# al-mcintyre/mCaller

Measured on NVIDIA B200. Metric: per-read site calls/sec, higher is better.
Workload: dtype f64

## Files before the change

### include/mcaller_b200.h

```cpp
#ifndef MCALLER_B200_H
#define MCALLER_B200_H

#include <stdint.h>

#ifdef __cplusplus
extern "C" {
#endif

#define MC_ABI_VERSION 3

#define MC_TILE_BYTES 3840
#define MC_TEXT_PAD 4096
#define MC_MAXK 8

enum {
    MC_OK = 0,
    MC_EINVAL = -1,
    MC_ECUDA = -2,
    MC_ECAPACITY = -3
};

typedef struct mc_refindex {
    int32_t n_contigs;
    int32_t k;
    const uint8_t *d_names;
    const int32_t *d_name_off;
    const int64_t *d_base;
    const int32_t *d_len;
    const uint32_t *d_site_fwd;
    const uint32_t *d_site_rev;
    const uint32_t *d_cand;
    const uint32_t *d_rank_fwd;
    const uint32_t *d_rank_rev;
    const uint8_t *d_bases;
    int64_t total_bits;
} mc_refindex;

typedef struct mc_record {
    uint32_t line_lo;
    uint16_t line_hi;
    uint16_t name_off;
    int32_t pos;
    int32_t event_idx;
    double diff;
    uint16_t name_len;
    uint16_t contig;
    uint8_t flags;
    uint8_t kbits_fwd;
    uint8_t kbits_rev;
    uint8_t pad;
} mc_record;

#define MC_RF_EQ 1u
#define MC_RF_CAND 2u
#define MC_RF_BADNUM 4u
#define MC_RF_BADIDX 8u
#define MC_RF_RAW 16u
#define MC_RF_NEWREAD 32u
#define MC_RF_SEGKNOWN 64u

enum {
    MC_C_LINES = 0,
    MC_C_KEPT,
    MC_C_RECORDS,
    MC_C_SHORT,
    MC_C_UNKNOWN_CONTIG,
    MC_C_NNN,
    MC_C_BADPOS,
    MC_C_LONGLINE,
    MC_C_OVERFLOW,
    MC_C_RUN_CURSOR,
    MC_C_QUIET,
    MC_C_COUNT = 16
};

typedef struct mc_call {
    int64_t read_off;
    double prob;
    double feat[MC_MAXK + 1];
    int32_t read_len;
    int32_t mpos;
    int32_t site;
    uint32_t close_rec;
    uint16_t win_contig;
    uint16_t chrom_contig;
    uint8_t kind;
    uint8_t rev;
    uint8_t n_empty;
    uint8_t empty_mask;
    uint8_t model_sel;
    uint8_t label;
    uint8_t err;
    uint8_t pad0;
    uint32_t seg;
    uint32_t pad1;
    uint32_t pad2;
} mc_call;

enum { MC_CALL = 0, MC_TOO_MANY_SKIPS = 1, MC_MULTI_M = 2, MC_NONE = 3  };
#define MC_CE_CONTEXT 1u
#define MC_CE_MODELKEY 2u
#define MC_CE_BADNUM 4u
#define MC_CE_COLUMN 8u
#define MC_CE_SPACING 16u

enum { MC_MLP = 0, MC_LR = 1, MC_GNB = 2, MC_RF = 3 };
enum { MC_ACT_IDENTITY = 0, MC_ACT_LOGISTIC = 1, MC_ACT_TANH = 2, MC_ACT_RELU = 3 };
typedef struct mc_model {
    int32_t kind;
    int32_t n_in;
    int32_t n_layers;
    int32_t hidden_act;
    int32_t sizes[8];
    const double *d_weights;
    const double *d_biases;
    int32_t n_trees;
    int32_t max_nodes;
    const int32_t *d_tree_off;
    const int32_t *d_left;
    const int32_t *d_right;
    const int32_t *d_feature;
    const double *d_threshold;
    const double *d_leaf_p1;
} mc_model;

typedef struct mc_qual_entry {
    uint64_t hash;
    uint32_t check;
    uint32_t len;
    double qual;
} mc_qual_entry;


int mc_version(void);
int mc_sizeof(int what);
const char *mc_last_error(void);

int mc_read_u64(const uint64_t *d_src, int64_t n, uint64_t *h_dst, void *stream);

int mc_scan(const uint8_t *d_text, int64_t nbytes, const mc_refindex *ref, int dense,
            mc_record *d_rec, int64_t rec_cap, uint32_t *d_tile_tab , uint32_t *d_run_tab ,
            uint64_t *d_counters, void *stream);

int mc_scan_run_len(int64_t nbytes);

int mc_scan_set_run_len(int run_len);

int64_t mc_num_tiles(int64_t nbytes);

int64_t mc_workspace_bytes(int64_t n);

int mc_order_records(const uint8_t *d_text, int64_t nbytes, const mc_refindex *ref, const uint32_t *d_tile_tab, int64_t n_tiles,
                     uint32_t *d_run_tab, int run_len, const mc_record *d_rec_in, int64_t rec_in_cap, const uint64_t *d_scan_counters,
                     mc_record *d_rec_out, int64_t rec_out_cap, uint64_t *d_n_out, uint32_t *d_seg_flags ,
                     uint32_t *d_run_first , void *d_ws, void *stream);

int mc_segment_reads(const uint8_t *d_text, mc_record *d_rec, const uint64_t *d_n_records, int64_t rec_cap,
                     uint32_t *d_seg_flags , const uint32_t *d_run_first, int64_t n_runs,
                     uint32_t *d_seg_start, uint64_t *d_nseg, void *d_ws, void *stream);

int mc_segment_quality(const uint8_t *d_text, const mc_record *d_rec, const uint32_t *d_seg_start, const uint64_t *d_nseg,
                       int64_t seg_cap, const mc_qual_entry *d_table, int64_t table_size, double *d_seg_qual, uint64_t *d_err,
                       void *stream);

int mc_build_windows(const mc_record *d_rec, const uint64_t *d_n_records, int64_t rec_cap, const uint32_t *d_seg_start,
                     const uint64_t *d_nseg, int64_t seg_cap, const double *d_seg_qual, const mc_refindex *ref, int skip_thresh,
                     double qual_thresh, int two_models, mc_call *d_calls, int64_t call_cap, uint32_t *d_seg_count,
                     uint64_t *d_ncalls, void *d_ws, double *d_spill, int64_t spill_cap, void *stream);

typedef struct mc_carry {
    mc_call row;
    uint32_t valid;
    int32_t first_kept_contig;
    uint64_t chunks;
    uint64_t pad[6];
} mc_carry;
int mc_carry_reset(mc_carry *d_carry, void *stream);
int mc_carry_rows(mc_call *d_rows, const uint64_t *d_ncalls, const mc_record *d_rec, const uint64_t *d_n_records,
                  const uint32_t *d_seg_start, const uint64_t *d_nseg, const double *d_seg_qual, double qual_thresh,
                  mc_carry *d_carry, uint64_t *d_nrows_out, const uint64_t *d_abort, void *stream);
int mc_chunk_guard(const uint64_t *d_counters, int64_t rec_cap, const uint64_t *d_n_records, int64_t rec_out_cap,
                   const uint64_t *d_nseg, int64_t seg_cap, const uint64_t *d_ncalls, int64_t call_cap, uint64_t *d_abort,
                   uint64_t *d_sticky , void *stream);
int mc_carry_close(mc_carry *d_carry, int closing_contig, const int64_t *d_next_contigs, int from, int count, mc_call *d_row_out,
                   uint32_t *d_depth, uint32_t *d_meth, uint64_t *d_first, int64_t n_sites, uint64_t *d_row_base, void *stream);

int64_t mc_classify_workspace_bytes(int64_t row_cap);
int mc_classify(mc_call *d_calls, const uint64_t *d_nrows, int64_t row_cap, const mc_model *models, void *d_ws, void *stream);

int mc_hist_accumulate(const mc_call *d_calls, const uint64_t *d_nrows, int64_t row_cap, uint32_t *d_depth, uint32_t *d_meth,
                       uint64_t *d_first, int64_t n_sites, uint64_t *d_row_base, mc_call *d_odd, int64_t odd_cap, uint64_t *d_n_odd,
                       const uint64_t *d_abort , void *stream);

int mc_bed_select(const uint32_t *d_depth, const uint32_t *d_meth, int64_t n_sites, int64_t depth_thresh, double mod_thresh,
                  int control, uint8_t *d_flags, uint64_t *d_count, void *stream);

int mc_count_calls(const mc_call *d_calls, const uint64_t *d_nrows, int64_t row_cap, uint64_t *d_out, void *stream);

typedef struct mc_locus_entry {
    unsigned long long hash;
// ... 83 lines not shown
```

### mcaller_b200/_lib.py

```python
import ctypes as C
import os

import numpy as np

HERE = os.path.dirname(os.path.abspath(__file__))
LIB_PATH = os.environ.get("MCALLER_B200_LIB") or os.path.join(HERE, "libmcaller_b200.so")

MC_TILE_BYTES = 3840
MC_TEXT_PAD = 4096
MC_MAXK = 8
MC_C_COUNT = 16
COUNTER_NAMES = ["lines", "kept", "records", "short", "unknown_contig", "nnn", "badpos", "longline", "overflow", "run_cursor", "quiet_chunks"]

MC_ABI_VERSION = 3
MC_CALL, MC_TOO_MANY_SKIPS, MC_MULTI_M, MC_NONE = 0, 1, 2, 3
MC_CE_CONTEXT, MC_CE_MODELKEY, MC_CE_BADNUM, MC_CE_COLUMN, MC_CE_SPACING = 1, 2, 4, 8, 16
MC_MLP, MC_LR, MC_GNB, MC_RF = 0, 1, 2, 3
PENDING = 0xFFFFFFFF


class RefIndex(C.Structure):
    _fields_ = [("n_contigs", C.c_int32), ("k", C.c_int32), ("d_names", C.c_void_p), ("d_name_off", C.c_void_p),
                ("d_base", C.c_void_p), ("d_len", C.c_void_p), ("d_site_fwd", C.c_void_p), ("d_site_rev", C.c_void_p),
                ("d_cand", C.c_void_p), ("d_rank_fwd", C.c_void_p), ("d_rank_rev", C.c_void_p), ("d_bases", C.c_void_p),
                ("total_bits", C.c_int64)]


class Model(C.Structure):
    _fields_ = [("kind", C.c_int32), ("n_in", C.c_int32), ("n_layers", C.c_int32), ("hidden_act", C.c_int32),
                ("sizes", C.c_int32 * 8), ("d_weights", C.c_void_p), ("d_biases", C.c_void_p), ("n_trees", C.c_int32),
                ("max_nodes", C.c_int32), ("d_tree_off", C.c_void_p), ("d_left", C.c_void_p), ("d_right", C.c_void_p),
                ("d_feature", C.c_void_p), ("d_threshold", C.c_void_p), ("d_leaf_p1", C.c_void_p)]


class SynthSpec(C.Structure):
    _fields_ = [("seed", C.c_uint64), ("n_contigs", C.c_int32), ("len_min", C.c_int32), ("len_max", C.c_int32),
                ("p_skip", C.c_int32), ("p_nnn", C.c_int32), ("margin", C.c_int32), ("meth", C.c_int32),
                ("d_names", C.c_void_p), ("d_name_off", C.c_void_p), ("d_contig_len", C.c_void_p),
                ("d_read_bounds", C.c_void_p), ("d_gbase", C.c_void_p), ("d_genome", C.c_void_p),
                ("d_meth_fwd", C.c_void_p), ("d_meth_rev", C.c_void_p), ("d_model_mean", C.c_void_p),
                ("d_model_sd", C.c_void_p)]


RECORD_DTYPE = np.dtype([("line_lo", "<u4"), ("line_hi", "<u2"), ("name_off", "<u2"), ("pos", "<i4"), ("event_idx", "<i4"),
                         ("diff", "<f8"), ("name_len", "<u2"), ("contig", "<u2"), ("flags", "u1"), ("kbits_fwd", "u1"), ("kbits_rev", "u1"), ("pad", "u1")])
assert RECORD_DTYPE.itemsize == 32

CALL_DTYPE = np.dtype([("read_off", "<i8"), ("prob", "<f8"), ("feat", "<f8", (MC_MAXK + 1,)), ("read_len", "<i4"),
                       ("mpos", "<i4"), ("site", "<i4"), ("close_rec", "<u4"), ("win_contig", "<u2"), ("chrom_contig", "<u2"),
                       ("kind", "u1"), ("rev", "u1"), ("n_empty", "u1"), ("empty_mask", "u1"), ("model_sel", "u1"),
                       ("label", "u1"), ("err", "u1"), ("pad0", "u1"), ("seg", "<u4"), ("pad1", "<u4"), ("pad2", "<u4")])
assert CALL_DTYPE.itemsize == 128

class LocusEntry(C.Structure):
    _fields_ = [("hash", C.c_uint64), ("first_off", C.c_uint64), ("check", C.c_uint64), ("depth", C.c_uint32), ("meth", C.c_uint32)]


class TrainJob(C.Structure):
    _fields_ = [("d_x", C.c_void_p), ("d_y", C.c_void_p), ("d_w", C.c_void_p), ("d_loss_curve", C.c_void_p), ("idx_off", C.c_int64),
                ("n", C.c_int32), ("d", C.c_int32), ("max_iter", C.c_int32), ("n_iter_no_change", C.c_int32), ("alpha", C.c_double),
                ("lr", C.c_double), ("tol", C.c_double), ("best_loss", C.c_double), ("n_iter", C.c_int32), ("no_improve", C.c_int32),
                ("stopped", C.c_int32), ("pad", C.c_int32)]


MC_TRAIN_HIDDEN, MC_TRAIN_BATCH = 100, 200

CARRY_BYTES = 192

QUAL_DTYPE = np.dtype([("hash", "<u8"), ("check", "<u4"), ("len", "<u4"), ("qual", "<f8")])
assert QUAL_DTYPE.itemsize == 24
DIFFS_ROW_DTYPE = np.dtype([("line_off", "<u8"), ("slot", "<u4"), ("values_off", "<u4"), ("values_len", "<u4"), ("prob_off", "<u4"),
                            ("prob_len", "<u4"), ("pad", "<u4")])
assert DIFFS_ROW_DTYPE.itemsize == 32


class McallerCudaError(RuntimeError):
    pass


_lib = None

_PROTOS = {
    "mc_version": (C.c_int, []),
    "mc_sizeof": (C.c_int, [C.c_int]),
    "mc_last_error": (C.c_char_p, []),
    "mc_read_u64": (C.c_int, [C.c_void_p, C.c_int64, C.c_void_p, C.c_void_p]),
    "mc_scan": (C.c_int, [C.c_void_p, C.c_int64, C.POINTER(RefIndex), C.c_int, C.c_void_p, C.c_int64, C.c_void_p, C.c_void_p, C.c_void_p,
                          C.c_void_p]),
    "mc_scan_run_len": (C.c_int, [C.c_int64]),
    "mc_scan_set_run_len": (C.c_int, [C.c_int]),
    "mc_num_tiles": (C.c_int64, [C.c_int64]),
    "mc_workspace_bytes": (C.c_int64, [C.c_int64]),
    "mc_order_records": (C.c_int, [C.c_void_p, C.c_int64, C.POINTER(RefIndex), C.c_void_p, C.c_int64, C.c_void_p, C.c_int, C.c_void_p,
                                   C.c_int64, C.c_void_p, C.c_void_p, C.c_int64, C.c_void_p, C.c_void_p, C.c_void_p, C.c_void_p, C.c_void_p]),
    "mc_segment_reads": (C.c_int, [C.c_void_p, C.c_void_p, C.c_void_p, C.c_int64, C.c_void_p, C.c_void_p, C.c_int64, C.c_void_p, C.c_void_p,
                                   C.c_void_p, C.c_void_p]),
    "mc_segment_quality": (C.c_int, [C.c_void_p, C.c_void_p, C.c_void_p, C.c_void_p, C.c_int64, C.c_void_p, C.c_int64, C.c_void_p,
                                     C.c_void_p, C.c_void_p]),
    "mc_build_windows": (C.c_int, [C.c_void_p, C.c_void_p, C.c_int64, C.c_void_p, C.c_void_p, C.c_int64, C.c_void_p, C.POINTER(RefIndex),
                                   C.c_int, C.c_double, C.c_int, C.c_void_p, C.c_int64, C.c_void_p, C.c_void_p, C.c_void_p, C.c_void_p,
                                   C.c_int64, C.c_void_p]),
    "mc_carry_reset": (C.c_int, [C.c_void_p, C.c_void_p]),
    "mc_carry_rows": (C.c_int, [C.c_void_p, C.c_void_p, C.c_void_p, C.c_void_p, C.c_void_p, C.c_void_p, C.c_void_p, C.c_double, C.c_void_p,
                                C.c_void_p, C.c_void_p, C.c_void_p]),
    "mc_chunk_guard": (C.c_int, [C.c_void_p, C.c_int64, C.c_void_p, C.c_int64, C.c_void_p, C.c_int64, C.c_void_p, C.c_int64, C.c_void_p,
                                 C.c_void_p, C.c_void_p]),
    "mc_carry_close": (C.c_int, [C.c_void_p, C.c_int, C.c_void_p, C.c_int, C.c_int, C.c_void_p, C.c_void_p, C.c_void_p, C.c_void_p,
                                 C.c_int64, C.c_void_p, C.c_void_p]),
    "mc_classify_workspace_bytes": (C.c_int64, [C.c_int64]),
    "mc_classify": (C.c_int, [C.c_void_p, C.c_void_p, C.c_int64, C.POINTER(Model), C.c_void_p, C.c_void_p]),
    "mc_hist_accumulate": (C.c_int, [C.c_void_p, C.c_void_p, C.c_int64, C.c_void_p, C.c_void_p, C.c_void_p, C.c_int64, C.c_void_p,
                                     C.c_void_p, C.c_int64, C.c_void_p, C.c_void_p, C.c_void_p]),
    "mc_count_calls": (C.c_int, [C.c_void_p, C.c_void_p, C.c_int64, C.c_void_p, C.c_void_p]),
    "mc_bed_select": (C.c_int, [C.c_void_p, C.c_void_p, C.c_int64, C.c_int64, C.c_double, C.c_int, C.c_void_p, C.c_void_p, C.c_void_p]),
    "mc_format_rows": (C.c_int64, [C.c_void_p, C.c_int64, C.c_void_p, C.c_void_p, C.c_int32, C.c_void_p, C.c_void_p, C.c_void_p, C.c_void_p,
                                   C.c_int32, C.c_int32, C.c_char_p, C.c_char_p, C.c_int32, C.c_int32, C.c_void_p, C.c_int64]),
    "mc_fastq_tiles": (C.c_int64, [C.c_int64]),
    "mc_fastq_index": (C.c_int, [C.c_void_p, C.c_int64, C.c_void_p, C.c_void_p, C.c_void_p, C.c_int64, C.c_void_p, C.c_void_p, C.c_void_p]),
    "mc_fastq_quality": (C.c_int, [C.c_void_p, C.c_int64, C.c_void_p, C.c_int64, C.c_void_p, C.c_int64, C.c_void_p, C.c_void_p, C.c_void_p,
                                   C.c_void_p]),
    "mc_synth_genome": (C.c_int, [C.POINTER(SynthSpec), C.c_void_p, C.c_int64, C.c_void_p]),
    "mc_synth_sizes": (C.c_int, [C.POINTER(SynthSpec), C.c_int64, C.c_int64, C.c_int64, C.c_void_p, C.c_void_p]),
    "mc_synth_write": (C.c_int, [C.POINTER(SynthSpec), C.c_int64, C.c_int64, C.c_int64, C.c_void_p, C.c_void_p, C.c_void_p]),
    "mc_diffs_aggregate_ex": (C.c_int, [C.c_void_p, C.c_int64, C.c_int64, C.c_void_p, C.c_int64, C.c_void_p, C.c_int64, C.c_void_p, C.c_void_p]),
    "mc_diffs_rehash": (C.c_int, [C.c_void_p, C.c_int64, C.c_void_p, C.c_int64, C.c_void_p, C.c_void_p]),
    "mc_diffs_rows": (C.c_int, [C.c_void_p, C.c_int64, C.c_void_p, C.c_int64, C.c_void_p, C.c_int64, C.c_void_p, C.c_int64, C.c_void_p,
                                C.c_void_p]),
    "mc_mlp_train_init": (C.c_int, [C.c_void_p, C.c_int32, C.c_void_p]),
    "mc_mlp_train_epochs": (C.c_int, [C.c_void_p, C.c_int32, C.c_void_p, C.c_int32, C.c_void_p]),
    "mc_diffs_colstats": (C.c_int, [C.c_void_p, C.c_void_p, C.c_void_p, C.c_int64, C.c_void_p, C.c_int64, C.c_int, C.c_void_p, C.c_void_p,
                                    C.c_void_p, C.c_void_p, C.c_void_p]),
}

EXPORTS = sorted(_PROTOS)


def load(path=LIB_PATH):
    if not os.path.exists(path):
        raise McallerCudaError("libmcaller_b200.so is not built (%s); run `python -m mcaller_b200.build` -- there is no CPU fallback" % path)
    lib = C.CDLL(path)
    for name, (res, args) in _PROTOS.items():
        fn = getattr(lib, name)
        fn.restype = res
# ... 17 lines not shown
```

### mcaller_b200/csrc/scan.cu

```cuda
#include "parse.cuh"

namespace {

constexpr int CHUNK = MC_TILE_BYTES;
constexpr int LOOKB = 32;
constexpr int LOOKA = 224;
constexpr int WB = LOOKB + CHUNK + LOOKA;
constexpr int NW = WB / 32;
#ifndef MC_SCAN_WARPS
#define MC_SCAN_WARPS 24
#endif
#ifndef MC_SCAN_MIN_CTAS
#define MC_SCAN_MIN_CTAS 1
#endif
#ifndef MC_SCAN_RUN
#define MC_SCAN_RUN 128
#endif

constexpr int WARPS = MC_SCAN_WARPS;
constexpr int THREADS = WARPS * 32;
constexpr int LCAP = 32;
constexpr int RESERVE = 256;
static_assert(WB == 4096 && NW == 128, "chunk geometry");
static_assert(CHUNK % 16 == 0, "chunks must keep 16-byte alignment");
// ... 163 lines not shown
    for (int j = 0; 8 * j < len; ++j) eq = eq && low_bytes(load8(text, qa + 8 * j) ^ load8(text, qb + 8 * j), len - 8 * j) == 0ull;
    return eq;
}
__device__ __forceinline__ int pos_digits8(unsigned long long k8) {
    const uint32_t lo = (uint32_t)k8, hi = (uint32_t)(k8 >> 32);
    const uint32_t xl = lo ^ 0x30303030u, xh = hi ^ 0x30303030u;
    const uint32_t ndl = (((xl & 0x7f7f7f7fu) + 0x76767676u) | lo) & 0x80808080u;
    const uint32_t ndh = (((xh & 0x7f7f7f7fu) + 0x76767676u) | hi) & 0x80808080u;
    return ndl ? ((__ffs(ndl) - 1) >> 3) : 4 + ((__ffs(ndh) - 1) >> 3);
}

enum { ST_KEPT = 1u, ST_CAND = 2u, ST_SHORT = 4u, ST_UNKNOWN = 8u, ST_NNN = 16u, ST_BADPOS = 32u };

template <class B>
__device__ __forceinline__ uint32_t classify_line(const B &t, int f0, int f1, int f9, const mc_refindex &R, int hint, int64_t hint_base,
                                                  int hint_len, int known_cid, int nnn_state ,
                                                  int pos_state , int &cid, int &pos) {
    cid = known_cid >= 0 ? known_cid : contig_lookup(t, f0, R, hint);
    if (cid < 0) return ST_UNKNOWN;
    if (nnn_state > 0 || (nnn_state < 0 && is_nnnnnn(t, f9))) return ST_NNN;
    if (pos_state == 0 || (pos_state < 0 && !parse_uint(t, f1, pos))) return ST_BADPOS;
    uint32_t st = ST_KEPT;
    const int len = (cid == hint) ? hint_len : __ldg(R.d_len + cid);
    if (pos < len) {
        const int64_t g = ((cid == hint) ? hint_base : __ldg(R.d_base + cid)) + pos;
        if ((__ldg(R.d_cand + (g >> 5)) >> (g & 31)) & 1u) st |= ST_CAND;
    }
    return st;
}

__device__ __noinline__ uint32_t classify_from_global(const uint8_t *d_text, int64_t limit, int64_t goff, const mc_refindex &R, int hint,
                                                      int64_t hint_base, int hint_len, int &cid, int &pos) {
    const GlobalBytes t{d_text + goff, limit - goff};
    int nf = 0, f0 = 0, f1 = 0, f9 = 0;
    bool in_tok = false;
    for (int i = 0; i < (1 << 20); ++i) {
        const int c = t[i];
        if (c == 0x0a) break;
        const bool ws = c <= 0x20;
        if (!ws && !in_tok) {
            if (nf == 0) f0 = i; else if (nf == 1) f1 = i; else if (nf == 9) f9 = i;
            ++nf;
            in_tok = true;
            if (nf >= 12) break;
        } else if (ws) in_tok = false;
    }
    if (nf < 12) return ST_SHORT;
    return classify_line(t, f0, f1, f9, R, hint, hint_base, hint_len, -1, -1, -1, cid, pos);
}

template <bool RF>
__global__ void __launch_bounds__(THREADS, MC_SCAN_MIN_CTAS)
k_scan(const uint8_t *__restrict__ d_text, int64_t nbytes, int64_t text_limit16, int64_t n_chunks64, int run_len, mc_refindex R,
       int dense, mc_record *__restrict__ d_rec, unsigned long long rec_cap, uint32_t *__restrict__ d_tile_tab,
       uint32_t *__restrict__ d_run_tab, unsigned long long *__restrict__ d_counters) {
    extern __shared__ __align__(16) uint8_t smem_raw[];
    const int lane = threadIdx.x & 31, wib = threadIdx.x >> 5;
    WarpSmem &S = reinterpret_cast<WarpSmem *>(smem_raw)[wib];
    const int warp_global = (int)blockIdx.x * WARPS + wib;
    const int n_warps = (int)gridDim.x * WARPS;
    const int n_chunks = (int)n_chunks64;
    const int n_runs = (n_chunks + run_len - 1) / run_len;
    const uint32_t lt_mask = (1u << lane) - 1u;

    const uint32_t K7F = 0x7f7f7f7fu | ((uint32_t)((unsigned long long)nbytes >> 63) << 7);
    auto eq0a_r = [&](uint32_t w) -> uint32_t {
        const uint32_t t = ((w ^ 0x0a0a0a0au) & K7F) + K7F;
        return ~(t | w) & 0x80808080u;
    };

    int hint = -1;
    int64_t hint_base = 0;
    int hint_len = 0, hint_nlen = 0;
    unsigned long long hint_key = 0ull;
    auto set_hint = [&](int c) {
        hint = c;
        hint_base = __ldg(R.d_base + c);
        hint_len = __ldg(R.d_len + c);
        const int o0 = __ldg(R.d_name_off + c);
        hint_nlen = __ldg(R.d_name_off + c + 1) - o0;
        hint_key = 0ull;
        for (int j = 0; j < hint_nlen && j < 7; ++j) hint_key |= (unsigned long long)__ldg(R.d_names + o0 + j) << (8 * j);
        __syncwarp();
        if (lane < 4) {
            unsigned long long kk = 0ull;
            for (int j = 8 * lane; j < hint_nlen && j < 8 * lane + 8; ++j) kk |= (unsigned long long)__ldg(R.d_names + o0 + j) << (8 * (j & 7));
            S.key[lane] = kk;
        }
        __syncwarp();
    };
    set_hint(0);
    unsigned long long slot_cur = 0ull;
    unsigned slot_left = 0u;
    unsigned c_lines = 0, c_kept = 0;
    if (lane < 8) S.cnt[lane] = 0u;

    if (lane == 0) {
        mbar_init(&S.bar[0], 1);
        mbar_init(&S.bar[1], 1);
        fence_barrier_init();
    }
    __syncwarp();
    uint32_t phase0 = 0u, phase1 = 0u;

    const int64_t q_hi = text_limit16 - WB + LOOKB, q_tail = nbytes - WB + LOOKB;
    const int c_bulk_hi = q_hi < 0 ? -1 : (int)min(q_hi / CHUNK, (int64_t)0x7fffffff);
    const int c_tail_lo = q_tail < 0 ? 0 : (int)min(q_tail / CHUNK + 1, (int64_t)0x7fffffff);
    auto stage = [&](int c, int b) -> bool {
        const int64_t g0 = (int64_t)c * CHUNK - LOOKB;
        if (c >= 1 && c <= c_bulk_hi) {
            if (lane == 0) {
                fence_proxy_async();
                tma_load_1d(S.text[b], d_text + g0, WB, &S.bar[b]);
            }
            return true;
        }
        for (int i = lane; i < WB / 16; i += 32) {
            const int64_t g = g0 + 16 * i;
            uint4 v = make_uint4(0x0a0a0a0au, 0x0a0a0a0au, 0x0a0a0a0au, 0x0a0a0a0au);
            if (g >= 0 && g < text_limit16) v = __ldg(reinterpret_cast<const uint4 *>(d_text + g));
            *reinterpret_cast<uint4 *>(S.text[b] + 16 * i) = v;
        }
        return false;
    };

    int rname_len = -1;
    auto rf_all_match = [&](const uint8_t *text, int nm) -> bool {
        const int j = lane & 15;
        const uint32_t kw = reinterpret_cast<const uint32_t *>(S.rname)[j];
        const int nb = rname_len - 4 * j;
        const uint32_t kmask = nb >= 4 ? 0xFFFFFFFFu : nb <= 0 ? 0u : ((1u << (8 * nb)) - 1u);
        const bool term_lane = j == (rname_len >> 2);
        const int term_sh = 8 * (rname_len & 3);
        const uint32_t *tw32 = reinterpret_cast<const uint32_t *>(text);
        uint32_t have = __ballot_sync(0xffffffffu, nm >= 0);
        while (have) {
            const int oa = __ffs(have) - 1;
            have &= have - 1u;
            const int ob = have ? __ffs(have) - 1 : -1;
            have &= have - 1u;
            const int o = lane < 16 ? oa : ob;
            const int a = __shfl_sync(0xffffffffu, nm, o < 0 ? 0 : o) + 4 * j;
            const uint32_t v = __funnelshift_r(tw32[a >> 2], tw32[(a >> 2) + 1], 8 * (a & 3));
            bool bad = ((v ^ kw) & kmask) != 0u;
            if (term_lane && ((v >> term_sh) & 0xFFu) > 0x20u) bad = true;
            if (o < 0) bad = false;
            if (__any_sync(0xffffffffu, bad)) return false;
        }
        return true;
    };

    int buf = 0;
    bool cur_async = false;
    int chunk = warp_global < n_runs ? warp_global * run_len : n_chunks;
    int run_end = min(chunk + run_len, n_chunks);
    if (chunk < n_chunks) cur_async = stage(chunk, 0);
    int prev_state = -1;
    bool read_has_kept = false;
    unsigned run_total = 0u, run_filler = 0u;

    while (chunk < n_chunks) {
        const int64_t G0 = (int64_t)chunk * CHUNK - LOOKB;
        const bool tail = chunk >= c_tail_lo;
        __syncwarp();
        int next = chunk + 1, next_end = run_end;
        const bool last_of_run = next >= run_end;
        if (last_of_run) {
            unsigned long long got = 0ull;
            if (lane == 0) got = atomicAdd(&d_counters[MC_C_RUN_CURSOR], 1ull);
            got = __shfl_sync(0xffffffffu, got, 0) + (unsigned long long)n_warps;
            next = got < (unsigned long long)n_runs ? (int)got * run_len : n_chunks;
            next_end = min(next + run_len, n_chunks);
        }
        bool next_async = false;
        if (next < n_chunks) next_async = stage(next, buf ^ 1);
        if (cur_async) {
            const uint32_t ph = buf ? phase1 : phase0;
            if (!mbar_wait(&S.bar[buf], ph) && lane == 0) atomicAdd(&S.cnt[5], 1u);
            if (buf) phase1 ^= 1u; else phase0 ^= 1u;
        }
        __syncwarp();
        const uint8_t *text = S.text[buf];
        const SmemBytes T{text};

#pragma unroll
        for (int r = 0; r < 4; ++r) {
            const int w = 32 * r + lane;
            const uint4 va = *reinterpret_cast<const uint4 *>(text + 32 * w);
            const uint4 vb = *reinterpret_cast<const uint4 *>(text + 32 * w + 16);
            S.nl[w] = pack32(eq0a_r(va.x), eq0a_r(va.y), eq0a_r(va.z), eq0a_r(va.w), eq0a_r(vb.x), eq0a_r(vb.y), eq0a_r(vb.z),
                             eq0a_r(vb.w));
        }
        if (lane == 0) S.nl[NW] = 0xFFFFFFFFu;
        __syncwarp();
        bool full_ready = false;

        uint4 lsv;
        {
            const uint4 nlv = *reinterpret_cast<const uint4 *>(&S.nl[4 * lane]);
            const uint32_t nprev = lane ? S.nl[4 * lane - 1] : 0u;
            lsv.x = (nlv.x << 1) | (nprev >> 31);
            lsv.y = (nlv.y << 1) | (nlv.x >> 31);
            lsv.z = (nlv.z << 1) | (nlv.y >> 31);
            lsv.w = (nlv.w << 1) | (nlv.z >> 31);
            constexpr int W_LO = LOOKB / 32, W_HI = (LOOKB + CHUNK) / 32;
            static_assert(W_LO == 1 && W_HI == 121, "the lane tests below assume words 1..120 are owned");
            const int w0 = 4 * lane;
            if (lane == 0) lsv.x = 0u;
            if (lane >= 30) {
                if (lane == 31) lsv.x = 0u;
                lsv.y = 0u; lsv.z = 0u; lsv.w = 0u;
            }
            if (tail) {
                auto clip = [&](uint32_t v, int w) {
                    const int64_t room = nbytes - (G0 + 32 * w);
                    return room <= 0 ? 0u : (room < 32 ? (v & ((1u << room) - 1u)) : v);
                };
                lsv.x = clip(lsv.x, w0);
                lsv.y = clip(lsv.y, w0 + 1);
                lsv.z = clip(lsv.z, w0 + 2);
                lsv.w = clip(lsv.w, w0 + 3);
            }
        }
        const int my_cnt = __popc(lsv.x) + __popc(lsv.y) + __popc(lsv.z) + __popc(lsv.w);
        c_lines += (unsigned)my_cnt;

        bool quiet_chunk = false;
        if (!dense && prev_state == 0 && hint_nlen >= 1 && hint_nlen <= 31 && (!RF || (read_has_kept && rname_len >= 1))) {
            uint32_t w0 = lsv.x, w1 = lsv.y, w2 = lsv.z, w3 = lsv.w;
            bool ok = true;
            int rf_round = 0, rf_nm1 = -1;
            for (;; ++rf_round) {
                if (!__any_sync(0xffffffffu, (w0 | w1 | w2 | w3) != 0u)) break;
                if ((w0 | w1 | w2 | w3) != 0u) {
                    const int jw = w0 ? 0 : w1 ? 1 : w2 ? 2 : 3;
                    const uint32_t m = w0 ? w0 : w1 ? w1 : w2 ? w2 : w3;
                    const int s0 = 32 * (4 * lane + jw) + __ffs(m) - 1;
                    const uint32_t cl = m & (m - 1u);
                    if (jw == 0) w0 = cl; else if (jw == 1) w1 = cl; else if (jw == 2) w2 = cl; else w3 = cl;
                    bool name_ok = true;
                    for (int j = 0; 8 * j <= hint_nlen; ++j) {
                        const unsigned long long v = load8(text, s0 + 8 * j), kk = S.key[j];
                        const int rem = hint_nlen - 8 * j;
                        if (rem >= 8) name_ok = name_ok && v == kk;
                        else name_ok = name_ok && (v & ((1ull << (8 * rem)) - 1ull)) == kk && ((v >> (8 * rem)) & 0xFFull) <= 0x20ull;
                    }
                    ok = false;
                    if (name_ok) {
                        int p0 = 0;
                        const unsigned long long p8 = load8(text, s0 + hint_nlen + 1);
                        if (parse_pos8(p8, p0) == 1) {
                            ok = true;
                            if (p0 < hint_len) {
                                const int64_t g = hint_base + p0;
                                ok = ((__ldg(R.d_cand + (g >> 5)) >> (g & 31)) & 1u) == 0u;
                            }
                            if (RF && ok) {
                                const int km = s0 + hint_nlen + 1 + pos_digits8(p8) + 1;
                                const unsigned long long k8 = load8(text, km);
                                const uint32_t wl = gt20_msb((uint32_t)k8) ^ 0x80808080u, wh = gt20_msb((uint32_t)(k8 >> 32)) ^ 0x80808080u;
                                const int klen = wl ? ((__ffs(wl) - 1) >> 3) : wh ? 4 + ((__ffs(wh) - 1) >> 3) : 8;
                                ok = klen >= 1 && klen <= 7 && rf_round < 2;
                                const int nm = km + klen + 1;
                                if (rf_round == 0) {
                                    const uint32_t *tw32 = reinterpret_cast<const uint32_t *>(text) + (nm >> 2);
                                    const uint32_t *kw32 = reinterpret_cast<const uint32_t *>(S.rname);
                                    const int sh = 8 * (nm & 3), nfull = rname_len >> 2;
                                    uint32_t prev = tw32[0], acc = 0u;
                                    for (int j = 0; j < nfull; ++j) {
                                        const uint32_t nxt = tw32[j + 1];
                                        acc |= __funnelshift_r(prev, nxt, sh) ^ kw32[j];
                                        prev = nxt;
                                    }
                                    const uint32_t v = __funnelshift_r(prev, tw32[nfull + 1], sh);
                                    const int nb = 8 * (rname_len & 3);
                                    acc |= (v ^ kw32[nfull]) & ((1u << nb) - 1u);
                                    ok = ok && acc == 0u && ((v >> nb) & 0xFFu) <= 0x20u;
                                } else {
                                    rf_nm1 = nm;
                                }
                            }
                        }
                    }
                }
                if (!__all_sync(0xffffffffu, ok)) { ok = false; break; }
            }
            if (RF && ok) ok = rf_all_match(text, rf_nm1);
            quiet_chunk = ok;
            if (ok && lane == 0) S.cnt[6] += 1u;
        }

        int my_first = 0, total_lines = 0;
        if (!quiet_chunk) {
            if (__ballot_sync(0xffffffffu, my_cnt > 3) == 0u) {
                const uint32_t b0 = __ballot_sync(0xffffffffu, my_cnt & 1), b1 = __ballot_sync(0xffffffffu, my_cnt & 2);
                my_first = __popc(b0 & lt_mask) + 2 * __popc(b1 & lt_mask);
                total_lines = __popc(b0) + 2 * __popc(b1);
            } else {
                int incl = my_cnt;
#pragma unroll
                for (int d = 1; d < 32; d <<= 1) {
                    const int tt = __shfl_up_sync(0xffffffffu, incl, d);
                    if (lane >= d) incl += tt;
                }
                total_lines = __shfl_sync(0xffffffffu, incl, 31);
                my_first = incl - my_cnt;
            }
            if (slot_left < (unsigned)total_lines) {
                unsigned long long got = 0ull;
                const unsigned want = total_lines > RESERVE ? (unsigned)total_lines : (unsigned)RESERVE;
                if (lane == 0) got = atomicAdd(&d_counters[MC_C_RECORDS], (unsigned long long)want);
                slot_cur = __shfl_sync(0xffffffffu, got, 0);
                slot_left = want;
            }
        }
        unsigned n_emitted = 0u;

        int e_last = -1;
        uint32_t filler = 0u;
        for (int pass0 = 0; pass0 < total_lines; pass0 += 32) {
            {
                int idx = my_first - pass0;
                uint32_t w0 = lsv.x, w1 = lsv.y, w2 = lsv.z, w3 = lsv.w;
                if (my_cnt <= 2) {
#pragma unroll
                    for (int t = 0; t < 2; ++t) {
                        if (t < my_cnt) {
                            const int jw = w0 ? 0 : w1 ? 1 : w2 ? 2 : 3;
                            const uint32_t m = w0 ? w0 : w1 ? w1 : w2 ? w2 : w3;
                            if (idx >= 0 && idx <= 32) S.lstart[idx] = (uint16_t)(32 * (4 * lane + jw) + __ffs(m) - 1);
                            ++idx;
                            const uint32_t cl = m & (m - 1u);
                            if (jw == 0) w0 = cl; else if (jw == 1) w1 = cl; else if (jw == 2) w2 = cl; else w3 = cl;
                        }
                    }
                } else {
                    const uint32_t wv[4] = {w0, w1, w2, w3};
#pragma unroll
                    for (int j = 0; j < 4; ++j) {
                        uint32_t m = wv[j];
                        while (m) {
                            const int b = __ffs(m) - 1;
                            m &= m - 1u;
                            if (idx >= 0 && idx <= 32) S.lstart[idx] = (uint16_t)(32 * (4 * lane + j) + b);
                            ++idx;
                        }
                    }
                }
            }
            __syncwarp();
            const int n_pass = min(32, total_lines - pass0);
            if (!full_ready) {
                full_ready = true;
                uint32_t prev_top = 0u;
#pragma unroll
                for (int r = 0; r < 4; ++r) {
                    const int w = 32 * r + lane;
                    const uint4 va = *reinterpret_cast<const uint4 *>(text + 32 * w);
                    const uint4 vb = *reinterpret_cast<const uint4 *>(text + 32 * w + 16);
                    const uint32_t nonws = pack32(gt20_msb(va.x), gt20_msb(va.y), gt20_msb(va.z), gt20_msb(va.w), gt20_msb(vb.x),
                                                  gt20_msb(vb.y), gt20_msb(vb.z), gt20_msb(vb.w));
                    const uint32_t top = nonws >> 31;
                    uint32_t pt = __shfl_up_sync(0xffffffffu, top, 1);
                    if (lane == 0) pt = prev_top;
                    prev_top = __shfl_sync(0xffffffffu, top, 31);
                    S.fs[w] = nonws & ~((nonws << 1) | pt);
                }
                if (lane < 8) S.fs[NW + lane] = 0u;
                if (!tail) {
                    constexpr int WLAST = (LOOKB + CHUNK - 1) >> 5, BLAST = (LOOKB + CHUNK - 1) & 31;
                    static_assert(NW - WLAST <= 32, "look-ahead words must fit one per lane");
                    int cand_e = NW * 32;
                    if (WLAST + lane < NW) {
                        uint32_t m = S.nl[WLAST + lane];
                        if (lane == 0) m &= 0xFFFFFFFFu << BLAST;
                        if (m) cand_e = 32 * (WLAST + lane) + __ffs(m) - 1;
                    }
                    e_last = __reduce_min_sync(0xffffffffu, cand_e);
                }
                __syncwarp();
            }
            uint32_t status = 0u;
            int cid = -1, pos = 0, s = 0;
            bool staged = false;
            int f3 = 0;
            if (lane < n_pass) {
                s = S.lstart[lane];
                const int e = (pass0 + lane + 1 < total_lines) ? (int)S.lstart[lane + 1] - 1 : (e_last >= 0 ? e_last : next_bit(S.nl, s));
                int f0, f1, f9, f11;
                line_fields<RF>(S, s, f0, f1, f9, f11, f3);
                if (f11 < e) {
                    staged = true;
                    const unsigned long long k8 = load8(text, f0);
                    const bool hit = hint_nlen <= 7 && (k8 & ((1ull << (8 * hint_nlen)) - 1ull)) == hint_key &&
                                     ((k8 >> (8 * hint_nlen)) & 0xFFull) <= 0x20ull;
                    int nnn = 0;
                    if (text[f9] == 'N') {
                        const unsigned long long m8 = load8(text, f9);
                        nnn = ((m8 & 0xFFFFFFFFFFFFull) == 0x4E4E4E4E4E4Eull && ((m8 >> 48) & 0xFFull) <= 0x20ull) ? 1 : 0;
                    }
                    const int pst = parse_pos8(load8(text, f1), pos);
                    status = classify_line(T, f0, f1, f9, R, hint, hint_base, hint_len, hit ? hint : -1, nnn, pst, cid, pos);
                } else if (e >= NW * 32 || f11 >= NW * 32) {
                    status = classify_from_global(d_text, nbytes + MC_TEXT_PAD - 64, G0 + s, R, hint, hint_base, hint_len, cid, pos);
                    atomicAdd(&S.cnt[4], 1u);
                } else {
                    status = ST_SHORT;
                }
            }
            if (status & (ST_SHORT | ST_UNKNOWN | ST_NNN | ST_BADPOS))
                atomicAdd(&S.cnt[(status & ST_SHORT) ? 0 : (status & ST_UNKNOWN) ? 1 : (status & ST_NNN) ? 2 : 3], 1u);

            const uint32_t kept_m = __ballot_sync(0xffffffffu, (status & ST_KEPT) != 0u);
            c_kept += (unsigned)__popc(kept_m);
            const uint32_t cand_m = __ballot_sync(0xffffffffu, (status & ST_CAND) != 0u);
            bool emit = false, filler_lane = false;
            if (RF) {
                const bool valid = lane < n_pass;
                const uint32_t unusual = __ballot_sync(0xffffffffu, valid && !staged);
                uint32_t new_m = 0u;
                if (unusual != 0u || rname_len < 1 || !rf_all_match(text, valid ? f3 : -1)) {
                int nq = 0, nlen = -1;
                if (valid && staged) {
                    nq = f3;
                    nlen = token_len64(text, nq);
                    if (nlen == 0) nlen = -1;
                }
                const int pq = __shfl_up_sync(0xffffffffu, nq, 1), plen = __shfl_up_sync(0xffffffffu, nlen, 1);
                bool same = false;
                if (valid && nlen > 0) {
                    if (lane == 0) same = nlen == rname_len && token_is(text, nq, nlen, S.rname);
                    else same = nlen == plen && spans_equal(text, nq, pq, nlen);
                }
                const uint32_t pass_m = n_pass >= 32 ? 0xFFFFFFFFu : ((1u << n_pass) - 1u);
                new_m = __ballot_sync(0xffffffffu, !same) & pass_m;
                const int lq = __shfl_sync(0xffffffffu, nq, n_pass - 1), llen = __shfl_sync(0xffffffffu, nlen, n_pass - 1);
                __syncwarp();
                if (llen > 0 && lane < 8) S.rname[lane] = 8 * lane < llen ? low_bytes(load8(text, lq + 8 * lane), llen - 8 * lane) : 0ull;
                rname_len = (llen > 0 && llen <= 63) ? llen : -1;
                __syncwarp();
                }
                if (status & ST_KEPT) {
                    const uint32_t nle = new_m & ((2u << lane) - 1u);
                    bool had;
                    if (nle == 0u) had = read_has_kept || (kept_m & lt_mask) != 0u;
                    else had = (kept_m & lt_mask & ~((1u << (31 - __clz(nle))) - 1u)) != 0u;
                    if (!had) emit = true;
                }
                if (new_m == 0u) read_has_kept = read_has_kept || kept_m != 0u;
                else read_has_kept = (kept_m >> (31 - __clz(new_m))) != 0u;
            }
            if (status & ST_KEPT) {
                if (dense || (status & ST_CAND)) emit = true;
                else {
                    const uint32_t below = kept_m & lt_mask;
                    const int st = below ? (int)((cand_m >> (31 - __clz(below))) & 1u) : prev_state;
                    if (st != 0) emit = true;
                    if (st < 0 && !RF) filler_lane = true;
                }
            }
            const uint32_t emit_m = __ballot_sync(0xffffffffu, emit);
            if (__ballot_sync(0xffffffffu, filler_lane)) filler = 1u;
// ... 18 lines not shown
                    } else {
                        fl |= 2u << 24;
                    }
                    const int64_t goff = G0 + s;
                    uint4 a, b;
                    a.x = (uint32_t)(goff & 0xFFFFFFFFll);
                    a.y = ((uint32_t)(goff >> 32) & 0xFFFFu) | (W3 << 16);
                    a.z = (uint32_t)pos;
                    a.w = W0;
                    b.x = W1; b.y = W2;
                    b.z = (W3 >> 16) | ((uint32_t)cid << 16);
                    b.w = fl;
                    uint4 *dst = reinterpret_cast<uint4 *>(d_rec + slot);
                    dst[0] = a;
                    dst[1] = b;
                } else {
                    atomicAdd(&S.cnt[5], 1u);
                }
            }
            {
                const unsigned ne = (unsigned)__popc(emit_m);
                slot_cur += ne;
                slot_left -= ne;
                n_emitted += ne;
            }
            __syncwarp();
        }
        if (lane == 0) {
            reinterpret_cast<uint2 *>(d_tile_tab)[chunk] =
                make_uint2((uint32_t)(slot_cur - n_emitted), n_emitted | (filler << 16) | ((uint32_t)(prev_state + 1) << 17));
        }
        run_total += n_emitted;
        run_filler |= filler;
        if (last_of_run) {
            if (lane == 0) reinterpret_cast<uint2 *>(d_run_tab)[chunk / run_len] = make_uint2(run_total, run_filler | ((uint32_t)(prev_state + 1) << 1));
            run_total = 0u;
            run_filler = 0u;
            prev_state = -1;
            rname_len = -1;
            read_has_kept = false;
        }
        chunk = next;
        run_end = next_end;
        buf ^= 1;
        cur_async = next_async;
    }

    __syncwarp();
    c_lines = __reduce_add_sync(0xffffffffu, c_lines);
    if (lane == 0) {
        if (c_lines) atomicAdd(&d_counters[MC_C_LINES], (unsigned long long)c_lines);
        if (c_kept) atomicAdd(&d_counters[MC_C_KEPT], (unsigned long long)c_kept);
        if (S.cnt[6]) atomicAdd(&d_counters[MC_C_QUIET], (unsigned long long)S.cnt[6]);
    }
    if (lane < 6) {
        const int which = lane == 0 ? MC_C_SHORT : lane == 1 ? MC_C_UNKNOWN_CONTIG : lane == 2 ? MC_C_NNN : lane == 3 ? MC_C_BADPOS
                        : lane == 4 ? MC_C_LONGLINE : MC_C_OVERFLOW;
        const unsigned v = S.cnt[lane];
        if (v) atomicAdd(&d_counters[which], (unsigned long long)v);
    }
}

}

static int g_run_len_override = 0;
extern "C" int mc_scan_set_run_len(int run_len) {
    const int before = g_run_len_override;
    g_run_len_override = run_len < 0 ? 0 : (run_len > 4096 ? 4096 : run_len);
    return before;
}

extern "C" int64_t mc_num_tiles(int64_t nbytes) { return nbytes <= 0 ? 0 : (nbytes + CHUNK - 1) / CHUNK; }

static int scan_geometry(int64_t n_chunks, int64_t *blocks_out, int *run_len_out) {
    int dev = 0, sms = 0;
    MC_CUDA_CHECK(cudaGetDevice(&dev));
    MC_CUDA_CHECK(cudaDeviceGetAttribute(&sms, cudaDevAttrMultiProcessorCount, dev));
    int64_t blocks = (n_chunks + WARPS - 1) / WARPS;
    const int64_t resident = (int64_t)sms * MC_SCAN_MIN_CTAS;
    if (blocks > resident) blocks = resident;
    int run_len = MC_SCAN_RUN;
    while (run_len > 1 && n_chunks < blocks * WARPS * 8 * (int64_t)run_len) run_len >>= 1;
    if (g_run_len_override > 0) run_len = g_run_len_override;
    *blocks_out = blocks;
    *run_len_out = run_len;
    return MC_OK;
}
extern "C" int mc_scan_run_len(int64_t nbytes) {
    const int64_t n_chunks = mc_num_tiles(nbytes);
    if (n_chunks == 0) return 1;
    int64_t blocks = 0;
    int run_len = 1;
    if (scan_geometry(n_chunks, &blocks, &run_len)) return -1;
    return run_len;
}

extern "C" int mc_scan(const uint8_t *d_text, int64_t nbytes, const mc_refindex *ref, int dense, mc_record *d_rec,
                       int64_t rec_cap, uint32_t *d_tile_tab, uint32_t *d_run_tab, uint64_t *d_counters, void *stream) {
    MC_REQUIRE(d_text && ref && d_rec && d_tile_tab && d_run_tab && d_counters, "null pointer");
    MC_REQUIRE(nbytes >= 0 && rec_cap >= 0, "negative size");
    MC_REQUIRE((reinterpret_cast<uintptr_t>(d_text) & 15) == 0, "d_text must be 16-byte aligned");
    MC_REQUIRE((reinterpret_cast<uintptr_t>(d_tile_tab) & 7) == 0, "d_tile_tab must be 8-byte aligned");
    MC_REQUIRE(ref->k >= 1 && ref->k <= MC_MAXK, "k out of range");
    MC_REQUIRE(ref->n_contigs >= 1 && ref->n_contigs < 65535, "contig count out of range");
    MC_REQUIRE(nbytes < (1ll << 47), "chunk too large");
    MC_REQUIRE(rec_cap < (1ll << 32), "record capacity must fit 32 bits");
    const int64_t n_chunks = mc_num_tiles(nbytes);
    if (n_chunks == 0) return MC_OK;
    MC_REQUIRE(n_chunks < (1ll << 30), "too many chunks (chunk of text larger than 4 TB)");
    const size_t smem = sizeof(WarpSmem) * WARPS;
    const bool read_first = dense == 2;
    MC_CUDA_CHECK(cudaFuncSetAttribute(read_first ? k_scan<true> : k_scan<false>, cudaFuncAttributeMaxDynamicSharedMemorySize, (int)smem));
    int64_t blocks = 0;
    int run_len = 1;
    {
        const int rc = scan_geometry(n_chunks, &blocks, &run_len);
        if (rc) return rc;
    }
    const int64_t text_limit16 = ((nbytes + MC_TEXT_PAD) / 16) * 16;
    MC_CUDA_CHECK(cudaMemsetAsync(d_counters + MC_C_RUN_CURSOR, 0, sizeof(uint64_t), (cudaStream_t)stream));
    if (read_first)
        k_scan<true><<<(unsigned)blocks, THREADS, smem, (cudaStream_t)stream>>>(d_text, nbytes, text_limit16, n_chunks, run_len, *ref, 0, d_rec,
                                                                               (unsigned long long)rec_cap, d_tile_tab, d_run_tab,
                                                                               reinterpret_cast<unsigned long long *>(d_counters));
    else
        k_scan<false><<<(unsigned)blocks, THREADS, smem, (cudaStream_t)stream>>>(d_text, nbytes, text_limit16, n_chunks, run_len, *ref, dense ? 1 : 0,
                                                                                d_rec, (unsigned long long)rec_cap, d_tile_tab, d_run_tab,
                                                                                reinterpret_cast<unsigned long long *>(d_counters));
    MC_LAUNCH_CHECK();
    return MC_OK;
}
```

Measured before the change: 49.74 million.

## Skip full line parsing on settled chunks, classifying only candidate-adjacent lines

```diff
diff --git a/include/mcaller_b200.h b/include/mcaller_b200.h
--- a/include/mcaller_b200.h
+++ b/include/mcaller_b200.h
@@ -71,6 +71,7 @@
     MC_C_OVERFLOW,
     MC_C_RUN_CURSOR,
     MC_C_QUIET,
+    MC_C_SETTLED,
     MC_C_COUNT = 16
 };
 
@@ -146,6 +147,8 @@
 
 int mc_scan_set_run_len(int run_len);
 
+int mc_scan_set_full_parse(int on);
+
 int64_t mc_num_tiles(int64_t nbytes);
 
 int64_t mc_workspace_bytes(int64_t n);
diff --git a/mcaller_b200/_lib.py b/mcaller_b200/_lib.py
--- a/mcaller_b200/_lib.py
+++ b/mcaller_b200/_lib.py
@@ -10,7 +10,7 @@
 MC_TEXT_PAD = 4096
 MC_MAXK = 8
 MC_C_COUNT = 16
-COUNTER_NAMES = ["lines", "kept", "records", "short", "unknown_contig", "nnn", "badpos", "longline", "overflow", "run_cursor", "quiet_chunks"]
+COUNTER_NAMES = ["lines", "kept", "records", "short", "unknown_contig", "nnn", "badpos", "longline", "overflow", "run_cursor", "quiet_chunks", "settled_chunks"]
 
 MC_ABI_VERSION = 3
 MC_CALL, MC_TOO_MANY_SKIPS, MC_MULTI_M, MC_NONE = 0, 1, 2, 3
@@ -89,6 +89,7 @@
                           C.c_void_p]),
     "mc_scan_run_len": (C.c_int, [C.c_int64]),
     "mc_scan_set_run_len": (C.c_int, [C.c_int]),
+    "mc_scan_set_full_parse": (C.c_int, [C.c_int]),
     "mc_num_tiles": (C.c_int64, [C.c_int64]),
     "mc_workspace_bytes": (C.c_int64, [C.c_int64]),
     "mc_order_records": (C.c_int, [C.c_void_p, C.c_int64, C.POINTER(RefIndex), C.c_void_p, C.c_int64, C.c_void_p, C.c_int, C.c_void_p,
diff --git a/mcaller_b200/csrc/scan.cu b/mcaller_b200/csrc/scan.cu
--- a/mcaller_b200/csrc/scan.cu
+++ b/mcaller_b200/csrc/scan.cu
@@ -239,7 +239,7 @@
 template <bool RF>
 __global__ void __launch_bounds__(THREADS, MC_SCAN_MIN_CTAS)
 k_scan(const uint8_t *__restrict__ d_text, int64_t nbytes, int64_t text_limit16, int64_t n_chunks64, int run_len, mc_refindex R,
-       int dense, mc_record *__restrict__ d_rec, unsigned long long rec_cap, uint32_t *__restrict__ d_tile_tab,
+       int dense, int settle, mc_record *__restrict__ d_rec, unsigned long long rec_cap, uint32_t *__restrict__ d_tile_tab,
        uint32_t *__restrict__ d_run_tab, unsigned long long *__restrict__ d_counters) {
     extern __shared__ __align__(16) uint8_t smem_raw[];
     const int lane = threadIdx.x & 31, wib = threadIdx.x >> 5;
@@ -281,6 +281,7 @@
     unsigned slot_left = 0u;
     unsigned c_lines = 0, c_kept = 0;
     if (lane < 8) S.cnt[lane] = 0u;
+    if (lane < 8) S.fs[NW + lane] = 0u;
 
     if (lane == 0) {
         mbar_init(&S.bar[0], 1);
@@ -288,7 +289,7 @@
         fence_barrier_init();
     }
     __syncwarp();
-    uint32_t phase0 = 0u, phase1 = 0u;
+    uint32_t phases = 0u;
 
     const int64_t q_hi = text_limit16 - WB + LOOKB, q_tail = nbytes - WB + LOOKB;
     const int c_bulk_hi = q_hi < 0 ? -1 : (int)min(q_hi / CHUNK, (int64_t)0x7fffffff);
@@ -362,9 +363,9 @@
         bool next_async = false;
         if (next < n_chunks) next_async = stage(next, buf ^ 1);
         if (cur_async) {
-            const uint32_t ph = buf ? phase1 : phase0;
+            const uint32_t ph = (phases >> buf) & 1u;
             if (!mbar_wait(&S.bar[buf], ph) && lane == 0) atomicAdd(&S.cnt[5], 1u);
-            if (buf) phase1 ^= 1u; else phase0 ^= 1u;
+            phases ^= 1u << buf;
         }
         __syncwarp();
         const uint8_t *text = S.text[buf];
@@ -380,7 +381,7 @@
         }
         if (lane == 0) S.nl[NW] = 0xFFFFFFFFu;
         __syncwarp();
-        bool full_ready = false;
+        uint32_t fs_built = 0u;
 
         uint4 lsv;
         {
@@ -412,8 +413,11 @@
         const int my_cnt = __popc(lsv.x) + __popc(lsv.y) + __popc(lsv.z) + __popc(lsv.w);
         c_lines += (unsigned)my_cnt;
 
-        bool quiet_chunk = false;
-        if (!dense && prev_state == 0 && hint_nlen >= 1 && hint_nlen <= 31 && (!RF || (read_has_kept && rname_len >= 1))) {
+        bool quiet_chunk = false, settled_chunk = false;
+        uint32_t ql_uns = 0u, ql_cand = 0u;
+        uint32_t cand_lines = 0u;
+        int e_last = -1;
+        if (!dense && hint_nlen >= 1 && hint_nlen <= 31 && (!RF || (prev_state == 0 && read_has_kept && rname_len >= 1))) {
             uint32_t w0 = lsv.x, w1 = lsv.y, w2 = lsv.z, w3 = lsv.w;
             bool ok = true;
             int rf_round = 0, rf_nm1 = -1;
@@ -433,11 +437,13 @@
                         else name_ok = name_ok && (v & ((1ull << (8 * rem)) - 1ull)) == kk && ((v >> (8 * rem)) & 0xFFull) <= 0x20ull;
                     }
                     ok = false;
+                    bool settled = false;
                     if (name_ok) {
                         int p0 = 0;
                         const unsigned long long p8 = load8(text, s0 + hint_nlen + 1);
                         if (parse_pos8(p8, p0) == 1) {
                             ok = true;
+                            settled = true;
                             if (p0 < hint_len) {
                                 const int64_t g = hint_base + p0;
                                 ok = ((__ldg(R.d_cand + (g >> 5)) >> (g & 31)) & 1u) == 0u;
@@ -469,10 +475,20 @@
                             }
                         }
                     }
-                }
-                if (!__all_sync(0xffffffffu, ok)) { ok = false; break; }
+                    if (!RF) {
+                        const uint32_t bit = 1u << min(rf_round, 31);
+                        if (!settled) ql_uns |= bit;
+                        else if (!ok) ql_cand |= bit;
+                    }
+                }
+                if (RF && !__all_sync(0xffffffffu, ok)) { ok = false; break; }
             }
             if (RF && ok) ok = rf_all_match(text, rf_nm1);
+            if (!RF) {
+                const bool all_settled = !__any_sync(0xffffffffu, ql_uns != 0u);
+                ok = all_settled && prev_state == 0 && !__any_sync(0xffffffffu, ql_cand != 0u);
+                settled_chunk = settle && all_settled && !ok;
+            }
             quiet_chunk = ok;
             if (ok && lane == 0) S.cnt[6] += 1u;
         }
@@ -500,10 +516,25 @@
                 slot_cur = __shfl_sync(0xffffffffu, got, 0);
                 slot_left = want;
             }
+            settled_chunk = settled_chunk && total_lines <= 32;
+            if (settled_chunk) {
+                cand_lines = __reduce_or_sync(0xffffffffu, my_first < 32 ? ql_cand << my_first : 0u);
+                if (lane == 0) S.cnt[7] += 1u;
+            }
+            if (!tail) {
+                constexpr int WLAST = (LOOKB + CHUNK - 1) >> 5, BLAST = (LOOKB + CHUNK - 1) & 31;
+                static_assert(NW - WLAST <= 32, "look-ahead words must fit one per lane");
+                int cand_e = NW * 32;
+                if (WLAST + lane < NW) {
+                    uint32_t m = S.nl[WLAST + lane];
+                    if (lane == 0) m &= 0xFFFFFFFFu << BLAST;
+                    if (m) cand_e = 32 * (WLAST + lane) + __ffs(m) - 1;
+                }
+                e_last = __reduce_min_sync(0xffffffffu, cand_e);
+            }
         }
         unsigned n_emitted = 0u;
 
-        int e_last = -1;
         uint32_t filler = 0u;
         for (int pass0 = 0; pass0 < total_lines; pass0 += 32) {
             {
@@ -537,64 +568,83 @@
             }
             __syncwarp();
             const int n_pass = min(32, total_lines - pass0);
-            if (!full_ready) {
-                full_ready = true;
-                uint32_t prev_top = 0u;
+            auto line_end = [&](int s) {
+                return (pass0 + lane + 1 < total_lines) ? (int)S.lstart[lane + 1] - 1 : (e_last >= 0 ? e_last : next_bit(S.nl, s));
+            };
+            uint32_t res = 0u;
+            int pos = 0;
+            int f3 = 0;
+            bool need = lane < n_pass;
+            for (;;) {
+                uint32_t rounds = 0xFu;
+                if (settled_chunk) {
+                    const uint32_t seen_m = __ballot_sync(0xffffffffu, res != 0u);
+                    const uint32_t kept_seen = __ballot_sync(0xffffffffu, (res & ST_KEPT) != 0u);
+                    const uint32_t maybe = (n_pass >= 32 ? 0xFFFFFFFFu : (1u << n_pass) - 1u) & ~(seen_m & ~kept_seen);
+                    const uint32_t below = maybe & lt_mask;
+                    const bool after_src = below ? ((cand_lines >> (31 - __clz(below))) & 1u) != 0u : prev_state != 0;
+                    need = ((maybe & ~seen_m) >> lane) & 1u;
+                    need = need && (((cand_lines >> lane) & 1u) || after_src || (maybe >> lane) == 1u);
+                    if (!__any_sync(0xffffffffu, need)) break;
+                    uint32_t my_rounds = 0u;
+                    if (need) {
+                        const int s0 = S.lstart[lane];
+                        my_rounds = (2u << min(max((s0 & ~31) + 191, line_end(s0)) >> 10, 3)) - (1u << (s0 >> 10));
+                    }
+                    rounds = __reduce_or_sync(0xffffffffu, my_rounds);
+                }
+                rounds &= ~fs_built;
+                if (rounds) {
+                    fs_built |= rounds;
 #pragma unroll
-                for (int r = 0; r < 4; ++r) {
-                    const int w = 32 * r + lane;
-                    const uint4 va = *reinterpret_cast<const uint4 *>(text + 32 * w);
-                    const uint4 vb = *reinterpret_cast<const uint4 *>(text + 32 * w + 16);
-                    const uint32_t nonws = pack32(gt20_msb(va.x), gt20_msb(va.y), gt20_msb(va.z), gt20_msb(va.w), gt20_msb(vb.x),
-                                                  gt20_msb(vb.y), gt20_msb(vb.z), gt20_msb(vb.w));
-                    const uint32_t top = nonws >> 31;
-                    uint32_t pt = __shfl_up_sync(0xffffffffu, top, 1);
-                    if (lane == 0) pt = prev_top;
-                    prev_top = __shfl_sync(0xffffffffu, top, 31);
-                    S.fs[w] = nonws & ~((nonws << 1) | pt);
-                }
-                if (lane < 8) S.fs[NW + lane] = 0u;
-                if (!tail) {
-                    constexpr int WLAST = (LOOKB + CHUNK - 1) >> 5, BLAST = (LOOKB + CHUNK - 1) & 31;
-                    static_assert(NW - WLAST <= 32, "look-ahead words must fit one per lane");
-                    int cand_e = NW * 32;
-                    if (WLAST + lane < NW) {
-                        uint32_t m = S.nl[WLAST + lane];
-                        if (lane == 0) m &= 0xFFFFFFFFu << BLAST;
-                        if (m) cand_e = 32 * (WLAST + lane) + __ffs(m) - 1;
+                    for (int r = 0; r < 4; ++r) {
+                        if ((rounds >> r) & 1u) {
+                            const int w = 32 * r + lane;
+                            const uint4 va = *reinterpret_cast<const uint4 *>(text + 32 * w);
+                            const uint4 vb = *reinterpret_cast<const uint4 *>(text + 32 * w + 16);
+                            const uint32_t nonws = pack32(gt20_msb(va.x), gt20_msb(va.y), gt20_msb(va.z), gt20_msb(va.w), gt20_msb(vb.x),
+                                                          gt20_msb(vb.y), gt20_msb(vb.z), gt20_msb(vb.w));
+                            uint32_t pt = __shfl_up_sync(0xffffffffu, nonws >> 31, 1);
+                            if (lane == 0) pt = r ? (text[1024 * r - 1] > 0x20 ? 1u : 0u) : 0u;
+                            S.fs[w] = nonws & ~((nonws << 1) | pt);
+                        }
                     }
-                    e_last = __reduce_min_sync(0xffffffffu, cand_e);
-                }
-                __syncwarp();
-            }
-            uint32_t status = 0u;
-            int cid = -1, pos = 0, s = 0;
-            bool staged = false;
-            int f3 = 0;
-            if (lane < n_pass) {
-                s = S.lstart[lane];
-                const int e = (pass0 + lane + 1 < total_lines) ? (int)S.lstart[lane + 1] - 1 : (e_last >= 0 ? e_last : next_bit(S.nl, s));
-                int f0, f1, f9, f11;
-                line_fields<RF>(S, s, f0, f1, f9, f11, f3);
-                if (f11 < e) {
-                    staged = true;
-                    const unsigned long long k8 = load8(text, f0);
-                    const bool hit = hint_nlen <= 7 && (k8 & ((1ull << (8 * hint_nlen)) - 1ull)) == hint_key &&
-                                     ((k8 >> (8 * hint_nlen)) & 0xFFull) <= 0x20ull;
-                    int nnn = 0;
-                    if (text[f9] == 'N') {
-                        const unsigned long long m8 = load8(text, f9);
-                        nnn = ((m8 & 0xFFFFFFFFFFFFull) == 0x4E4E4E4E4E4Eull && ((m8 >> 48) & 0xFFull) <= 0x20ull) ? 1 : 0;
+                    __syncwarp();
+                }
+                if (need) {
+                    const int s = S.lstart[lane];
+                    const int e = line_end(s);
+                    uint32_t status;
+                    int cid = -1;
+                    bool staged = false;
+                    int f0, f1, f9, f11;
+                    line_fields<RF>(S, s, f0, f1, f9, f11, f3);
+                    if (f11 < e) {
+                        staged = true;
+                        const unsigned long long k8 = load8(text, f0);
+                        const bool hit = hint_nlen <= 7 && (k8 & ((1ull << (8 * hint_nlen)) - 1ull)) == hint_key &&
+                                         ((k8 >> (8 * hint_nlen)) & 0xFFull) <= 0x20ull;
+                        int nnn = 0;
+                        if (text[f9] == 'N') {
+                            const unsigned long long m8 = load8(text, f9);
+                            nnn = ((m8 & 0xFFFFFFFFFFFFull) == 0x4E4E4E4E4E4Eull && ((m8 >> 48) & 0xFFull) <= 0x20ull) ? 1 : 0;
+                        }
+                        const int pst = parse_pos8(load8(text, f1), pos);
+                        status = classify_line(T, f0, f1, f9, R, hint, hint_base, hint_len, hit ? hint : -1, nnn, pst, cid, pos);
+                    } else if (e >= NW * 32 || f11 >= NW * 32) {
+                        status = classify_from_global(d_text, nbytes + MC_TEXT_PAD - 64, G0 + s, R, hint, hint_base, hint_len, cid, pos);
+                        atomicAdd(&S.cnt[4], 1u);
+                    } else {
+                        status = ST_SHORT;
                     }
-                    const int pst = parse_pos8(load8(text, f1), pos);
-                    status = classify_line(T, f0, f1, f9, R, hint, hint_base, hint_len, hit ? hint : -1, nnn, pst, cid, pos);
-                } else if (e >= NW * 32 || f11 >= NW * 32) {
-                    status = classify_from_global(d_text, nbytes + MC_TEXT_PAD - 64, G0 + s, R, hint, hint_base, hint_len, cid, pos);
-                    atomicAdd(&S.cnt[4], 1u);
-                } else {
-                    status = ST_SHORT;
-                }
-            }
+                    res = status | (staged ? 64u : 0u) | ((uint32_t)cid << 16);
+                }
+                if (!settled_chunk) break;
+            }
+            const uint32_t status = res & 63u;
+            const bool staged = (res & 64u) != 0u;
+            const int cid = (int)(res >> 16);
+            const int s = lane < n_pass ? (int)S.lstart[lane] : 0;
             if (status & (ST_SHORT | ST_UNKNOWN | ST_NNN | ST_BADPOS))
                 atomicAdd(&S.cnt[(status & ST_SHORT) ? 0 : (status & ST_UNKNOWN) ? 1 : (status & ST_NNN) ? 2 : 3], 1u);
 
@@ -719,6 +769,7 @@
         if (c_lines) atomicAdd(&d_counters[MC_C_LINES], (unsigned long long)c_lines);
         if (c_kept) atomicAdd(&d_counters[MC_C_KEPT], (unsigned long long)c_kept);
         if (S.cnt[6]) atomicAdd(&d_counters[MC_C_QUIET], (unsigned long long)S.cnt[6]);
+        if (S.cnt[7]) atomicAdd(&d_counters[MC_C_SETTLED], (unsigned long long)S.cnt[7]);
     }
     if (lane < 6) {
         const int which = lane == 0 ? MC_C_SHORT : lane == 1 ? MC_C_UNKNOWN_CONTIG : lane == 2 ? MC_C_NNN : lane == 3 ? MC_C_BADPOS
@@ -734,6 +785,13 @@
 extern "C" int mc_scan_set_run_len(int run_len) {
     const int before = g_run_len_override;
     g_run_len_override = run_len < 0 ? 0 : (run_len > 4096 ? 4096 : run_len);
+    return before;
+}
+
+static int g_full_parse = 0;
+extern "C" int mc_scan_set_full_parse(int on) {
+    const int before = g_full_parse;
+    g_full_parse = on ? 1 : 0;
     return before;
 }
 
@@ -787,11 +845,12 @@
     const int64_t text_limit16 = ((nbytes + MC_TEXT_PAD) / 16) * 16;
     MC_CUDA_CHECK(cudaMemsetAsync(d_counters + MC_C_RUN_CURSOR, 0, sizeof(uint64_t), (cudaStream_t)stream));
     if (read_first)
-        k_scan<true><<<(unsigned)blocks, THREADS, smem, (cudaStream_t)stream>>>(d_text, nbytes, text_limit16, n_chunks, run_len, *ref, 0, d_rec,
+        k_scan<true><<<(unsigned)blocks, THREADS, smem, (cudaStream_t)stream>>>(d_text, nbytes, text_limit16, n_chunks, run_len, *ref, 0, 0, d_rec,
                                                                                (unsigned long long)rec_cap, d_tile_tab, d_run_tab,
                                                                                reinterpret_cast<unsigned long long *>(d_counters));
     else
         k_scan<false><<<(unsigned)blocks, THREADS, smem, (cudaStream_t)stream>>>(d_text, nbytes, text_limit16, n_chunks, run_len, *ref, dense ? 1 : 0,
+                                                                                g_full_parse ? 0 : 1,
                                                                                 d_rec, (unsigned long long)rec_cap, d_tile_tab, d_run_tab,
                                                                                 reinterpret_cast<unsigned long long *>(d_counters));
     MC_LAUNCH_CHECK();
```

Result: slower. 40.68 million (median of 6 runs) (-18.2%).
